# harshadms/galileo-sdr-sim

Measured on AMD Instinct MI355X. Metric: IQ Msamples/s (×real-time @2.6MS/s), 12-SV static E1B/C, 1/2/4/8 GPU, higher is better.
Workload: dtype f64 (NCO phases) + int16x2 (packed accumulate) -> int16 IQ; 1 GPU; M-SYN12: static-geometry 12-SV E1B/C, 1199 epochs x 260000 samples @2.6 MS/s per GPU (one independent scenario per rank); channels=12, chunk_samples=1024, walk_passes=1, synth_runs_max=1, chain_mismatch=0, pipeline_depth=2, window_mode=1, kernel_family=1, output_checksum=26e91314

## Files before the change

galileo-sdr-sim_amd/csrc/synth_api.cpp:

```cpp
#include <hip/hip_runtime.h>

#include <algorithm>
#include <cmath>
#include <cstdarg>
#include <cstddef>
#include <type_traits>
#include <cstdio>
#include <cstdlib>
#include <cstring>
#include <new>
#include <chrono>
#include <sched.h>
#include <time.h>
#include <vector>

#define GAL_SYNTH_NO_SIZED_MACROS 1
#include "nco_walk.h"
#include "synth_dev.h"
#include "e1_tables.inc"

static double rw_threshold_edge(double s)
{
    double g = 1.0;
    for (int u = 1; u <= 15; ++u) {
        const double us = (double)u * s;
        const double t = 1.0 - (us - std::floor(us));
        g = std::min(g, std::min(t, 1.0 - t));
    }
    return g;
}

static double rw_threshold_gap(double s)
{
    double T[15];
    for (int u = 1; u <= 15; ++u) {
        const double us = (double)u * s;
        const double t = 1.0 - (us - std::floor(us));
        int i = u - 1;
        while (i > 0 && T[i - 1] > t) { T[i] = T[i - 1]; --i; }
        T[i] = t;
    }
    double g = 1.0;
    for (int i = 1; i < 15; ++i) g = std::min(g, T[i] - T[i - 1]);
    return g;
}
static int rw_mode_of(double cs2)
{
    return (cs2 >= 0.74 && cs2 < 0.9999) ? 1 : (cs2 >= 0.0083 && cs2 <= 0.133) ? 2 : (cs2 > 0.133 && cs2 <= 0.266) ? 3
           : (cs2 > 0.266 && cs2 < 0.74) ? 4 : 0;
}
static constexpr double kRwMinGap = 1.0 / 128.0 + 4e-6;
static constexpr double kRwMinGapCboc = 1.0 / 64.0 + 4e-6;
#ifdef GAL_TEST_HOOKS
extern "C" double gal_hooks_rw_threshold_gap(double s) { return rw_threshold_gap(s); }
extern "C" double gal_hooks_rw_min_gap(void) { return kRwMinGap; }
#endif

extern "C" {
void galk_warm(hipStream_t st, int signal, double ratio);
void galk_warm_g(hipStream_t st);
int galk_launch_synth_g(const DevPlan *P, const DevPlan *Pd, int nch, int accumulate, const uint8_t *act, const int *nact,
                        uint32_t *iq, int e0, int ne, hipStream_t st);
void galk_launch_repair_g(const DevPlan *P, uint32_t *iq, int e0, hipStream_t st);
void galk_touch(hipStream_t st);
void galk_launch_walk_code(const DevPlan *P, hipStream_t st);
void galk_launch_walk_carr(const DevPlan *P, int first, hipStream_t st);
void galk_launch_carr_scan(const DevPlan *P, uint32_t tag, hipStream_t st);
size_t galk_scanm_status_bytes(int S, int legs);
void galk_launch_verify_carr(const DevPlan *P, hipStream_t st);
void galk_launch_verify_code(const DevPlan *P, hipStream_t st);
void galk_launch_pages(const DevPlan *P, hipStream_t st);
void galk_launch_publish(const DevPlan *P, int *h_ctr, void *h_state, uint32_t *h_flag, uint32_t seq, hipStream_t st);
int galk_scanm_blocks(int legs);
size_t galk_scanm_bytes(int S, int legs);
int galk_launch_synth(const DevPlan *P, const DevPlan *Pd, int nch, int accumulate, const uint8_t *act,
                      const int *nact, uint32_t *iq, int e0, int ne, hipStream_t st);
hipError_t galk_launch_iq(int format, const int16_t *in, uint64_t n_val, int shift, void *out, unsigned long long *sat, hipStream_t st);
hipError_t galk_launch_iq_noise(int format, const int16_t *in, uint64_t n_val, uint64_t first_sample, uint64_t seed, uint32_t stream,
                                uint32_t gain_q16, uint32_t sigma_q4, int shift, void *out, unsigned long long *sat, hipStream_t st);
}

namespace {

thread_local char g_err[512] = "";

int fail(int code, const char *fmt, ...)
{
    va_list ap;
    va_start(ap, fmt);
    vsnprintf(g_err, sizeof(g_err), fmt, ap);
    va_end(ap);
    return code;
}

#define HIP_TRY(expr)                                                                              \
    do {                                                                                           \
        hipError_t err__ = (expr);                                                                 \
        if (err__ != hipSuccess)                                                                   \
            return fail(GAL_E_DEVICE, "%s failed: %s (%s:%d)", #expr, hipGetErrorString(err__),   \
                        __FILE__, __LINE__);                                                       \
    } while (0)

int16_t g_cos[512], g_sin[512];
bool g_tables_ready = false;

void init_tables()
{
    if (g_tables_ready) return;
    for (int k = 0; k < 512; ++k) {
        int q;
        if (k < 128) q = kCosQ[k];
        else if (k < 256) q = -kCosQ[255 - k];
        else if (k < 384) q = -kCosQ[k - 256];
        else q = kCosQ[511 - k];
        g_cos[k] = (int16_t)q;
    }
    for (int k = 0; k < 512; ++k) g_sin[k] = g_cos[(k - 128) & 511];
    g_tables_ready = true;
}

constexpr int kKernelMaxChan = 12;
constexpr size_t kRunHostStagedBytes = 32u << 20;
constexpr int kActRow = 32;
// ... 25 lines not shown
        const double d = galnco::eff_step(dstep);
        const double mine = reset ? (restart ? p0 : start_in) : ph;
        const double full = (double)N * d;
        double y = mine + (full - std::trunc(full));
        y = y - std::trunc(y);
        const bool mixed = mine != 0.0 && d != 0.0 && ((mine < 0.0) != (d < 0.0));
        const bool crossed = !mixed || std::fabs(full) > std::fabs(mine);
        if (y != 0.0 && d != 0.0) {
            const bool neg = crossed ? d < 0.0 : mine < 0.0;
            if ((y < 0.0) != neg) y += neg ? -1.0 : 1.0;
        }
        ph = y;
        const bool use_root = reset || kind != 1;
        *pguess = mine;
        *gss_w = use_root ? (long long)e * N : ev_w;
        *gss_r = use_root ? mine : ev_r;
        int om;
        double rr;
        if (galnco::ideal_last_wrap(mine, d, N, &om, &rr)) {
            kind = 1;
            ev_w = (long long)e * N + om;
            ev_r = rr;
        } else if (reset) {
            kind = 1;
            ev_w = (long long)e * N;
            ev_r = mine;
        }
    }
};

struct StagedPlan {
    DevPlan P{};
    int n_groups = 0, all_first = 0, all_count = 0, n_exact_records = 0, nact_max = 0;
    std::vector<int> group_nch, group_kind;
    std::vector<int64_t> act_prefix;
    size_t o_plan = 0, o_act = 0, o_nact = 0, up_bytes = 0, total = 0;
    size_t o_cpx = 0, o_ancw = 0, zero_end = 0, o_clmw = 0, clmw_bytes = 0, o_scanm = 0, scanm_clear = 0;
    int R = 0, nchunks = 0;
    float ms_plan = 0.0f;
};

struct gal_synth {
    StagedPlan staged;
    bool staged_pending = false;
    gal_synth_cfg_t cfg{};
    int device = 0;
    int n_cu = 256;
    hipStream_t own_stream = nullptr;
    hipStream_t stream = nullptr;
    hipStream_t aux_stream = nullptr;
    hipStream_t walk_stream = nullptr;
    hipEvent_t ev_walk = nullptr;
    hipEvent_t ev_ver = nullptr;
    hipEvent_t ev_verc = nullptr;
    hipEvent_t ev_ctr = nullptr;
    hipEvent_t ev[4] = {nullptr, nullptr, nullptr, nullptr};
    hipEvent_t ev_prep = nullptr, ev_aux = nullptr;
    hipEvent_t ev_upd = nullptr;

    int *d_lut = nullptr;
    uint32_t *d_str = nullptr;
    DevPlan *d_plan = nullptr;
    char *h_up = nullptr;
    size_t h_up_bytes = 0;

    void *arena = nullptr;
    size_t arena_bytes = 0;
    DevPlan P{};
    DevPlan Pw{};
    bool planned = false;
    bool executed = false;
    bool in_flight = false;
    int n_groups = 0;
    std::vector<int> group_nch;
    std::vector<int> group_kind;
    int all_first = 0, all_count = 0;
    int n_exact_records = 0;
    uint8_t *d_act = nullptr;
    int *d_nact = nullptr;
    int nact_max = 0;
    uint32_t *last_iq = nullptr;
    int range_e0 = 0, range_ne = 0;
    void *own_iq = nullptr;
    size_t own_iq_bytes = 0;
    void *own_pin = nullptr;
    size_t own_pin_bytes = 0;
    int *h_ctr = nullptr;
    uint32_t *h_flag = nullptr;
    uint32_t seq = 0;
    uint32_t scan_tag = 0;
    size_t scanm_off = ~(size_t)0, scanm_clear = 0;
    int64_t legs_walked = 0, legs_translated = 0, n_fallbacks = 0;
    std::vector<int64_t> act_prefix;
    int64_t first_pass_legs = 0;
    gal_chan_state_t *h_state = nullptr;
    bool state_fetched = false;
    gal_synth_stats_t stats{};
    int enq_passes = kDefaultPasses;
    int small_need = 2;
    std::vector<double> rw_s0, rw_g0, rw_e0;
    std::vector<double> rw_rad;
    bool host_only = false;
    hipEvent_t ev_up0 = nullptr, ev_up1 = nullptr;
    bool upload_pending = false;
    bool upload_timed = false;
    bool upload_unordered = false;
    float ms_plan = 0.0f;
    double prev_wait_us = 0.0;
// ... 72 lines not shown

    int ndev = 0;
    if (hipGetDeviceCount(&ndev) != hipSuccess || ndev < 1)
        return fail(GAL_E_DEVICE, "no HIP device: the synthesis engine has no CPU fallback");
    create_stage("hipGetDeviceCount (HIP start-up)");
    int dev = cfg->device;
    if (dev < 0) HIP_TRY(hipGetDevice(&dev));
    if (dev >= ndev) return fail(GAL_E_INVAL, "device %d out of range (%d devices)", dev, ndev);
    HIP_TRY(hipSetDevice(dev));
    hipDeviceProp_t prop;
    HIP_TRY(hipGetDeviceProperties(&prop, dev));
    if (!strstr(prop.gcnArchName, "gfx950"))
        return fail(GAL_E_DEVICE, "device %d is %s; this library carries gfx950 code only", dev,
                    prop.gcnArchName);

    create_stage("set device + properties");
    gal_synth *h = new (std::nothrow) gal_synth();
    if (!h) return fail(GAL_E_NOMEM, "out of host memory");
    h->cfg = *cfg;
    h->device = dev;
    h->n_cu = prop.multiProcessorCount > 0 ? prop.multiProcessorCount : 256;
    auto bail = [&](int code) {
        gal_synth_destroy(h);
        return code;
    };
    {
        bool have = false;
        if (!(cfg->flags & GAL_CFG_SINGLE_STREAM)) {
            int least = 0, greatest = 0;
            hipStream_t ws = nullptr, as = nullptr;
            if (hipDeviceGetStreamPriorityRange(&least, &greatest) == hipSuccess &&
                hipStreamCreateWithPriority(&ws, hipStreamNonBlocking, greatest) == hipSuccess &&
                hipStreamCreateWithPriority(&as, hipStreamNonBlocking, greatest) == hipSuccess &&
                hipEventCreateWithFlags(&h->ev_walk, hipEventDisableTiming) == hipSuccess) {
                h->walk_stream = ws;
                h->aux_stream = as;
                have = true;
            } else {
                (void)hipGetLastError();
                if (ws) hipStreamDestroy(ws);
                if (as) hipStreamDestroy(as);
            }
        }
        if (!have && hipStreamCreateWithFlags(&h->aux_stream, hipStreamNonBlocking) != hipSuccess)
            return bail(fail(GAL_E_DEVICE, "hipStreamCreate failed"));
    }
    create_stage("streams");
    for (auto &e : h->ev)
        if (hipEventCreate(&e) != hipSuccess) return bail(fail(GAL_E_DEVICE, "hipEventCreate failed"));
    if (hipEventCreate(&h->ev_up0) != hipSuccess || hipEventCreate(&h->ev_up1) != hipSuccess ||
        hipEventCreateWithFlags(&h->ev_prep, hipEventDisableTiming) != hipSuccess ||
        hipEventCreateWithFlags(&h->ev_upd, hipEventDisableTiming) != hipSuccess ||
        hipEventCreateWithFlags(&h->ev_ver, hipEventDisableTiming) != hipSuccess ||
        hipEventCreateWithFlags(&h->ev_verc, hipEventDisableTiming) != hipSuccess ||
        hipEventCreateWithFlags(&h->ev_ctr, hipEventDisableTiming) != hipSuccess ||
        hipEventCreateWithFlags(&h->ev_aux, hipEventDisableTiming) != hipSuccess)
        return bail(fail(GAL_E_DEVICE, "hipEventCreate failed"));
    if (hipHostMalloc((void **)&h->h_ctr, (2 * CTR_COUNT + 16) * sizeof(int), hipHostMallocCoherent) != hipSuccess ||
        hipHostMalloc((void **)&h->h_state, sizeof(gal_chan_state_t) * GAL_ENGINE_MAX_CHAN,
                      hipHostMallocCoherent) != hipSuccess)
        return bail(fail(GAL_E_NOMEM, "pinned host allocation failed"));
    h->h_flag = (uint32_t *)(h->h_ctr + 2 * CTR_COUNT);
    *h->h_flag = 0;

    create_stage("events + pinned record");
    if (hipMalloc((void **)&h->d_lut, 2 * 512 * sizeof(int)) != hipSuccess ||
        hipMalloc((void **)&h->d_str, 50 * 512 * sizeof(uint32_t)) != hipSuccess)
        return bail(fail(GAL_E_NOMEM, "table allocation failed"));
    {
        std::vector<uint32_t> str(50 * 512, 0u);
        for (int prn = 0; prn < 50; ++prn)
            for (int hc = 0; hc < 2 * GAL_CODE_LEN; ++hc) {
                const int chip = hc >> 1;
                const uint32_t b = (kE1B[prn][chip >> 5] >> (chip & 31)) & 1u, c = (kE1C[prn][chip >> 5] >> (chip & 31)) & 1u;
                const uint32_t two = (b ^ c) | ((c ^ (uint32_t)(hc & 1)) << 1);
                str[prn * 512 + (hc >> 4)] |= two << (2 * (hc & 15));
            }
        if (hipMemcpy(h->d_str, str.data(), str.size() * sizeof(uint32_t), hipMemcpyHostToDevice) != hipSuccess)
            return bail(fail(GAL_E_DEVICE, "table upload failed"));
    }
    int lut[2 * 512];
    auto pair = [](int c, int s) {
        return (int)(((uint32_t)(uint16_t)(int16_t)(2 * s) << 16) | (uint32_t)(uint16_t)(int16_t)(2 * c));
    };
    if (cfg->flags & GAL_CFG_CBOC) {
        const double alpha = std::sqrt(10.0 / 11.0), beta = std::sqrt(1.0 / 11.0);
        for (int k = 0; k < 512; ++k) {
            lut[k] = pair((int)std::lround(alpha * (double)g_cos[k]), (int)std::lround(alpha * (double)g_sin[k]));
            lut[512 + k] = pair((int)std::lround(beta * (double)g_cos[k]), (int)std::lround(beta * (double)g_sin[k]));
        }
    } else {
        for (int k = 0; k < 512; ++k) lut[k] = lut[512 + k] = pair(g_cos[k], g_sin[k]);
    }
    if (hipMemcpy(h->d_lut, lut, sizeof(lut), hipMemcpyHostToDevice) != hipSuccess)
        return bail(fail(GAL_E_DEVICE, "table upload failed"));
    create_stage("tables (hipMalloc + uploads)");
    galk_warm(nullptr, (cfg->flags & GAL_CFG_CBOC) ? 1 : 0, 2.0 * 1.023e6 / cfg->sample_rate);
    {
        const double ratio = 2.0 * 1.023e6 / cfg->sample_rate;
        bool g_possible = false;
        for (const double f : {1.0 - 1e-4, 1.0, 1.0 + 1e-4}) {
            const int m = rw_mode_of(ratio * f);
            g_possible = g_possible || m != 0;
        }
        if (g_possible && !(cfg->flags & GAL_CFG_EXACT_REPLAY) && cfg->chunk_samples <= 0) galk_warm_g(nullptr);
    }
    create_stage("warm launches enqueued");
    if (h->walk_stream) {
        galk_touch(h->walk_stream);
        galk_touch(h->aux_stream);
        if (hipStreamSynchronize(h->walk_stream) != hipSuccess || hipStreamSynchronize(h->aux_stream) != hipSuccess) {
            gal_synth_destroy(h);
            return fail(GAL_E_DEVICE, "kernel launch failed on device %d: %s", dev, hipGetErrorString(hipGetLastError()));
        }
    }
    if (hipStreamSynchronize(nullptr) != hipSuccess) {
        gal_synth_destroy(h);
        return fail(GAL_E_DEVICE, "kernel launch failed on device %d: %s", dev, hipGetErrorString(hipGetLastError()));
    }
    create_stage("code objects loaded, streams used");
#ifdef GAL_TEST_HOOKS
    if (const char *env = getenv("GAL_SCAN_TAG0")) h->scan_tag = (uint32_t)strtoul(env, nullptr, 0);
#endif
    *out = h;
    return GAL_OK;
}

int gal_synth_destroy(gal_synth_t *h)
{
    if (!h) return GAL_OK;
    hipSetDevice(h->device);
    if (h->stream) hipStreamSynchronize(h->stream);
    if (h->arena) hipFree(h->arena);
    if (h->own_iq) hipFree(h->own_iq);
    if (h->own_pin) hipHostFree(h->own_pin);
    if (h->d_iq_sat) hipFree(h->d_iq_sat);
    if (h->d_lut) hipFree(h->d_lut);
    if (h->d_str) hipFree(h->d_str);
    if (h->h_up) hipHostFree(h->h_up);
    if (h->h_ctr) hipHostFree(h->h_ctr);
    if (h->h_state) hipHostFree(h->h_state);
    for (auto &e : h->ev)
        if (e) hipEventDestroy(e);
    if (h->ev_prep) hipEventDestroy(h->ev_prep);
    if (h->ev_upd) hipEventDestroy(h->ev_upd);
    if (h->ev_up0) hipEventDestroy(h->ev_up0);
    if (h->ev_up1) hipEventDestroy(h->ev_up1);
    if (h->ev_aux) hipEventDestroy(h->ev_aux);
    if (h->ev_walk) hipEventDestroy(h->ev_walk);
    if (h->ev_ver) hipEventDestroy(h->ev_ver);
    if (h->ev_verc) hipEventDestroy(h->ev_verc);
    if (h->ev_ctr) hipEventDestroy(h->ev_ctr);
    if (h->walk_stream) hipStreamDestroy(h->walk_stream);
    if (h->aux_stream) hipStreamDestroy(h->aux_stream);
    if (h->own_stream) hipStreamDestroy(h->own_stream);
    delete h;
    return GAL_OK;
}

int gal_synth_set_stream(gal_synth_t *h, void *hip_stream)
{
    if (!h) return fail(GAL_E_INVAL, "null handle");
    h->stream = hip_stream ? (hipStream_t)hip_stream : h->own_stream;
    return GAL_OK;
}

size_t gal_synth_output_bytes(const gal_synth_t *h)
{
    if (!h) return 0;
    if (h->staged_pending) return (size_t)h->staged.P.E * (size_t)h->staged.P.N * 4u;
    if (!h->planned) return 0;
    return (size_t)h->P.E * (size_t)h->P.N * 4u;
}

static size_t align_up(size_t v, size_t a) { return (v + a - 1) / a * a; }

static int commit_staged(gal_synth *h, const bool wait)
{
    StagedPlan &sp = h->staged;
    if (!h->host_only && sp.total > h->arena_bytes) {
        if (h->arena) hipFree(h->arena);
        h->arena = nullptr;
        h->arena_bytes = 0;
        if (hipMalloc(&h->arena, sp.total) != hipSuccess) return fail(GAL_E_NOMEM, "hipMalloc of %zu bytes failed", sp.total);
        h->arena_bytes = sp.total;
        h->scanm_off = ~(size_t)0;
    }
    char *const base = (char *)h->arena;
    DevPlan &P = sp.P;
    {
        auto rb = [&](auto *&ptr) { ptr = (std::remove_reference_t<decltype(ptr)>)(base + (size_t)(uintptr_t)ptr); };
        rb(P.page_init); rb(P.init_ix); rb(P.state_in); rb(P.state_out); rb(P.prn); rb(P.flags); rb(P.ib0); rb(P.x0); rb(P.p0);
        rb(P.cstep); rb(P.dstep); rb(P.page_next); rb(P.page_cur); rb(P.flip_in); rb(P.pguess); rb(P.gss_w); rb(P.gss_r);
        rb(P.anc_w); rb(P.anc_r); rb(P.clm_w); rb(P.clm_r); rb(P.pend); rb(P.verified); rb(P.dirty); rb(P.risk); rb(P.marg);
        rb(P.shift); rb(P.tpos); rb(P.tdir); rb(P.scanm); rb(P.cp_x); rb(P.cp_p); rb(P.cp_ib); rb(P.ctr); rb(P.gflist);
    }
    h->P = P;
    h->d_plan = (DevPlan *)(base + sp.o_plan);
    h->d_act = (uint8_t *)(base + sp.o_act);
    h->d_nact = (int *)(base + sp.o_nact);
    h->n_groups = sp.n_groups; h->all_first = sp.all_first; h->all_count = sp.all_count; h->n_exact_records = sp.n_exact_records;
    h->group_nch = std::move(sp.group_nch);
    h->group_kind = std::move(sp.group_kind);
    h->act_prefix = std::move(sp.act_prefix);
    h->nact_max = sp.nact_max;
// ... 471 lines not shown
int gal_synth_plan_async(gal_synth_t *h, const gal_chan_epoch_t *params, int32_t n_epochs, const gal_chan_state_t *state_in)
{
    return plan_impl(h, params, n_epochs, state_in, false);
}

#ifdef GAL_TEST_HOOKS
static gal_synth *g_host_plan = nullptr;
double gal_hooks_plan_host_ms(const gal_synth_cfg_t *cfg, const gal_chan_epoch_t *params, int32_t n_epochs, const gal_chan_state_t *state_in,
                              int32_t reps)
{
    gal_synth *&g = g_host_plan;
    if (g) {
        free(g->h_up);
        delete g;
        g = nullptr;
    }
    if (!cfg || !params) return -1.0;
    g = new gal_synth();
    g->cfg = *cfg;
    g->host_only = true;
    init_tables();
    double best = 1e30;
    for (int r = 0; r < (reps > 0 ? reps : 1); ++r) {
        const auto t0 = std::chrono::steady_clock::now();
        if (plan_impl(g, params, n_epochs, state_in, false) != GAL_OK) return -1.0;
        best = std::min(best, std::chrono::duration<double, std::milli>(std::chrono::steady_clock::now() - t0).count());
    }
    return best;
}
const void *gal_hooks_plan_host_array(const char *name)
{
    const gal_synth *g = g_host_plan;
    if (!g || !g->planned || !name) return nullptr;
    const DevPlan &P = g->P;
    const struct { const char *n; const void *p; } tab[] = {
        {"prn", P.prn}, {"flags", P.flags}, {"ib0", P.ib0}, {"x0", P.x0}, {"p0", P.p0}, {"cstep", P.cstep}, {"dstep", P.dstep},
        {"page_next", P.page_next}, {"pguess", P.pguess}, {"gss_w", P.gss_w}, {"gss_r", P.gss_r}, {"init_ix", P.init_ix},
        {"page_init", P.page_init}, {"state_in", P.state_in}, {"act", g->d_act}, {"nact", g->d_nact}};
    for (const auto &t : tab)
        if (!strcmp(t.n, name)) return g->h_up + (size_t)(uintptr_t)t.p;
    if (!strcmp(name, "family")) return (const void *)(uintptr_t)(1 + P.fam);
    if (!strcmp(name, "groups")) return (const void *)(uintptr_t)(1 + g->n_groups);
    if (!strcmp(name, "search")) return (const void *)(uintptr_t)(1 + P.rw_search);
    if (!strcmp(name, "form")) return (const void *)(uintptr_t)(1 + P.rw);
    return nullptr;
}
#endif

static int enqueue_synth(gal_synth *h, uint32_t *iq, bool verify_here)
{
    if (verify_here && h->P.fam == 1 && h->nact_max != 0) {
        DevPlan Pv = h->Pw;
        if (h->stats.synth_runs > 1) Pv.ver_mod = 1, Pv.ver_rem = 0;
        galk_launch_verify_carr(&Pv, h->stream);
        galk_launch_verify_code(&Pv, h->stream);
    }
    if (h->nact_max == 0) {
        HIP_TRY(hipMemsetAsync(iq, 0, (size_t)h->range_ne * (size_t)h->P.N * 4u, h->stream));
        return GAL_OK;
    }
    const bool overflow_set = h->P.fam == 0 && h->all_count > 0;
    const int g_first = overflow_set ? h->all_first : 0, g_count = overflow_set ? h->all_count : h->n_groups;
    DevPlan Px = h->P;
    if (h->P.fam == 1 || overflow_set) Px.rw = 0;
    for (int k = 0; k < g_count; ++k) {
        const int g = g_first + k;
        const uint8_t *act = h->d_act + (size_t)g * h->P.E * kActRow;
        const int *nact = h->d_nact + (size_t)g * h->P.E;
        const bool on_g = h->P.fam == 1 && h->group_kind[g] == 1;
        const int rc = on_g ? galk_launch_synth_g(&h->P, h->d_plan, h->group_nch[g], k > 0, act, nact, iq, h->range_e0, h->range_ne, h->stream)
                            : galk_launch_synth(h->P.fam == 1 || overflow_set ? &Px : &h->P, h->d_plan, h->group_nch[g], k > 0, act, nact, iq,
                                                h->range_e0, h->range_ne, h->stream);
        if (rc) return fail(GAL_E_INVAL, "no synthesis kernel for %d channels per group", h->group_nch[g]);
    }
    if (h->P.fam == 1) {
        HIP_TRY(hipEventRecord(h->ev[3], h->stream));
        galk_launch_repair_g(&h->P, iq, h->range_e0, h->stream);
    }
    HIP_TRY(hipGetLastError());
    return GAL_OK;
}

static int ensure_committed(gal_synth *h)
{
    if (!h->staged_pending) return GAL_OK;
    if (h->in_flight) return fail(GAL_E_STATE, "gal_synth_execute while a batch is in flight: call gal_synth_finish first");
    HIP_TRY(hipSetDevice(h->device));
    return commit_staged(h, false);
}

int gal_synth_execute(gal_synth_t *h, int16_t *iq_dev)
{
    if (!h) return fail(GAL_E_INVAL, "gal_synth_execute: null argument");
    if (const int rc = ensure_committed(h)) return rc;
    if (!h->planned) return fail(GAL_E_STATE, "gal_synth_execute before gal_synth_plan");
    return gal_synth_execute_range(h, iq_dev, 0, h->P.E);
}

int gal_synth_execute_range(gal_synth_t *h, int16_t *iq_dev, int32_t first_epoch, int32_t n_epochs)
{
    if (!h || !iq_dev) return fail(GAL_E_INVAL, "gal_synth_execute: null argument");
    if (const int rc = ensure_committed(h)) return rc;
    if (!h->planned) return fail(GAL_E_STATE, "gal_synth_execute before gal_synth_plan");
    if (first_epoch < 0 || n_epochs < 1 || first_epoch + n_epochs > h->P.E)
        return fail(GAL_E_INVAL, "gal_synth_execute_range: epochs [%d, %d) outside the planned batch of %d", first_epoch,
                    first_epoch + n_epochs, h->P.E);
    if (h->in_flight)
        return fail(GAL_E_STATE, "gal_synth_execute while a batch is in flight: call gal_synth_finish first");
    if (((uintptr_t)iq_dev) & 15) return fail(GAL_E_INVAL, "iq_dev must be 16-byte aligned");
    HIP_TRY(hipSetDevice(h->device));
    if (h->executed && (first_epoch != h->range_e0 || n_epochs != h->range_ne)) h->enq_passes = std::max(h->enq_passes, kDefaultPasses);
    h->range_e0 = first_epoch;
    h->range_ne = n_epochs;
    h->Pw = h->P;
    h->Pw.E = first_epoch + n_epochs;
    h->Pw.LEGS = h->Pw.E * h->P.W;
    h->Pw.tr_e0 = first_epoch;
    h->Pw.tr_e1 = first_epoch + n_epochs;
    h->Pw.cp_e0 = first_epoch;
    h->Pw.ver_mod = (h->cfg.flags & GAL_CFG_VERIFY_SAMPLED) ? kVerifyRotation : 1;
#ifdef GAL_TEST_HOOKS
    if (const char *env = getenv("GAL_VERIFY_MOD")) h->Pw.ver_mod = atoi(env) > 0 ? atoi(env) : h->Pw.ver_mod;
#endif
    h->Pw.ver_rem = (int)((h->seq + 1u) % (uint32_t)h->Pw.ver_mod);
    hipStream_t st = handle_stream(h);
    if (!st) return fail(GAL_E_DEVICE, "hipStreamCreate failed");
    const DevPlan *P = &h->Pw;
    hipStream_t ws = h->walk_stream ? h->walk_stream : st;
    if (h->upload_unordered) {
        if (ws != st) HIP_TRY(hipStreamWaitEvent(ws, h->ev_upd, 0));
        h->upload_unordered = false;
    }
    HIP_TRY(hipEventRecord(h->ev[0], ws));
    HIP_TRY(hipEventRecord(h->ev_prep, ws));
    const bool code_first = h->Pw.E * 8 < 256 && h->aux_stream && h->aux_stream != ws;
    if (code_first) {
        HIP_TRY(hipStreamWaitEvent(h->aux_stream, h->ev_prep, 0));
        galk_launch_walk_code(P, h->aux_stream);
        galk_launch_pages(P, h->aux_stream);
        HIP_TRY(hipEventRecord(h->ev_aux, h->aux_stream));
    }
    int n_passes = h->enq_passes;
#ifdef GAL_TEST_HOOKS
    if (const char *env = getenv("GAL_WALK_PASSES")) n_passes = atoi(env) > 0 ? atoi(env) : n_passes;
#endif
    h->first_pass_legs = h->act_prefix[h->Pw.E] * h->P.W;
    if (h->scan_tag > 0xFFF00000u) {
        HIP_TRY(hipMemsetAsync((char *)h->P.scanm, 0, h->scanm_clear, ws));
        h->scan_tag = 0;
    }
    for (int pass = 0; pass < n_passes; ++pass) {
        galk_launch_walk_carr(P, pass == 0, ws);
        if (pass == 0 && ws != st) HIP_TRY(hipEventRecord(h->ev_ctr, ws));
        galk_launch_carr_scan(P, ++h->scan_tag, ws);
    }
    if (!code_first) {
        HIP_TRY(hipStreamWaitEvent(h->aux_stream, h->ev_prep, 0));
        galk_launch_walk_code(P, h->aux_stream);
        galk_launch_pages(P, h->aux_stream);
        HIP_TRY(hipEventRecord(h->ev_aux, h->aux_stream));
    }
    bool verify_beside = h->P.fam == 1 && ws != st && h->nact_max != 0;
#ifdef GAL_TEST_HOOKS
    const bool no_verify = getenv("GAL_G_NOVERIFY") != nullptr;
    if (no_verify) verify_beside = false;
#else
    const bool no_verify = false;
#endif
    if (ws != st) {
        HIP_TRY(hipEventRecord(h->ev_walk, ws));
        HIP_TRY(hipStreamWaitEvent(st, h->ev_walk, 0));
        if (verify_beside) {
            galk_launch_verify_carr(P, ws);
            HIP_TRY(hipEventRecord(h->ev_ver, ws));
            HIP_TRY(hipStreamWaitEvent(h->aux_stream, h->ev_ctr, 0));
            galk_launch_verify_code(P, h->aux_stream);
            HIP_TRY(hipEventRecord(h->ev_verc, h->aux_stream));
        }
    }
    HIP_TRY(hipStreamWaitEvent(st, h->ev_aux, 0));
    HIP_TRY(hipEventRecord(h->ev[1], st));
    int rc = enqueue_synth(h, (uint32_t *)iq_dev, !verify_beside && !no_verify);
    if (rc) return rc;
    HIP_TRY(hipEventRecord(h->ev[2], st));
    if (verify_beside) {
        HIP_TRY(hipStreamWaitEvent(st, h->ev_ver, 0));
        HIP_TRY(hipStreamWaitEvent(st, h->ev_verc, 0));
    }
    h->seq += 1;
    if (h->seq == 0) h->seq = 1;
    galk_launch_publish(P, h->h_ctr, h->h_state, h->h_flag, h->seq, st);
    h->state_fetched = true;
    h->last_iq = (uint32_t *)iq_dev;
    h->stats.synth_runs = 1;
    h->executed = true;
    h->in_flight = true;
    return GAL_OK;
}

size_t gal_synth_stats_size(void) { return sizeof(gal_synth_stats_t); }

static void copy_stats(const gal_synth *h, void *stats, size_t stats_bytes)
{
    if (stats) memcpy(stats, &h->stats, std::min(stats_bytes, sizeof(gal_synth_stats_t)));
}

static constexpr size_t kStatsBytesV02 = 40;
static_assert(offsetof(gal_synth_stats_t, kernel_family) == kStatsBytesV02, "gal_synth_stats_t 0.2 ends in front of kernel_family");

int gal_synth_finish(gal_synth_t *h, gal_chan_state_t *state_out, gal_synth_stats_t *stats)
{
    return gal_synth_finish_n(h, state_out, stats, kStatsBytesV02);
}

int gal_synth_finish_n(gal_synth_t *h, gal_chan_state_t *state_out, void *stats, size_t stats_bytes)
{
    if (!h) return fail(GAL_E_INVAL, "null handle");
    if (!h->executed) return fail(GAL_E_STATE, "gal_synth_finish before gal_synth_execute");
    h->in_flight = false;
    HIP_TRY(hipSetDevice(h->device));
    hipStream_t st = handle_stream(h);
    if (!st) return fail(GAL_E_DEVICE, "hipStreamCreate failed");
    const DevPlan *P = &h->Pw;
    {
        const uint32_t want = h->seq;
        const auto t_begin = std::chrono::steady_clock::now();
        unsigned spins = 0;
        double waited_us = 0.0;
        const double nap_until_us = 0.7 * h->prev_wait_us - 150.0;
        while (__atomic_load_n(h->h_flag, __ATOMIC_ACQUIRE) != want) {
            const bool look = (++spins & 255u) == 0;
            if (!look) {
                __builtin_ia32_pause();
                continue;
            }
            waited_us = std::chrono::duration<double, std::micro>(std::chrono::steady_clock::now() - t_begin).count();
            bool napped = false;
            if (waited_us >= 50.0) {
                if (waited_us < nap_until_us) {
                    timespec ts{0, 50000};
                    nanosleep(&ts, nullptr);
// ... 325 lines not shown
```

galileo-sdr-sim_amd/csrc/synth_kernels.hip:

```cpp
#include <hip/hip_runtime.h>
#include <stdint.h>

#include "nco_walk.h"
#include "synth_dev.h"
#include "synth_common.h"

using namespace galnco;
using namespace galdev;

#if !defined(GAL_TU)
#define GAL_TU_WALK 1
#define GAL_TU_SYNTH 1
#define GAL_TU_FAMILY(k) 1
#else
#define GAL_TU_WALK (GAL_TU == 0)
#define GAL_TU_SYNTH (GAL_TU != 0)
#define GAL_TU_FAMILY(k) (GAL_TU == (k))
#endif

#ifndef GAL_WALK_PRIO
#define GAL_WALK_PRIO 3
#endif
#if GAL_WALK_PRIO > 0
#define GAL_WALK_SETPRIO() __builtin_amdgcn_s_setprio(GAL_WALK_PRIO)
#else
#define GAL_WALK_SETPRIO() ((void)0)
#endif

#ifdef GAL_TEST_HOOKS
#define GAL_HOOK_BAD_LEG 5
#endif

#if GAL_TU_WALK
__device__ __forceinline__ double shfl_up1_f64(double v)
{
    const uint64_t u = d2u(v);
    const uint32_t lo = (uint32_t)__shfl_up((int)(uint32_t)u, 1), hi = (uint32_t)__shfl_up((int)(uint32_t)(u >> 32), 1);
    return u2d(((uint64_t)hi << 32) | lo);
}

__global__ void k_walk_code(DevPlan P)
{
    GAL_WALK_SETPRIO();
    const int Wc = P.Wc;
    const int t = blockIdx.x * blockDim.x + threadIdx.x;
    if (t >= P.E * P.S * Wc) return;
    const int k = t & (Wc - 1);
    const int se = t / Wc;
    const int s = se / P.E;
    const int idx = (se - s * P.E) * P.S + s;
    if (P.prn[idx] <= 0) return;
    double *cpx = P.cp_x + (size_t)idx * P.CP1;
    uint32_t *cpi = P.cp_ib + (size_t)idx * P.CP1;
    const double c = P.cstep[idx];
// ... 197 lines not shown
                for (int q = 0; q < 8; ++q) v[q] = P.dstep[(size_t)(e2 + q) * P.S + s];
                bool still = true;
#pragma unroll
                for (int q = 0; q < 8; ++q) still = still && v[q] == 0.0;
                if (!still) break;
                e2 += 8;
            }
            const long long skip_to = e2 * P.N;
            cur = skip_to < A ? skip_to : A;
            continue;
        }
        const WalkOut o = carr_walk_track(p, d, 1.0 / __builtin_fabs(d), n, n, n, [](int, double) {});
        if (o.last_w >= 0) {
            lw = cur + o.last_w;
            lr = o.last_r;
        }
        mg = o.margin < mg ? o.margin : mg;
        if (!tdir && o.tdir) {
            tdir = o.tdir;
            tpos = cur + o.tpos;
        }
        p = o.p;
        cur = seg_end;
    }
    int n = P.N - w * L;
    n = n > L ? L : n;
    const double d = P.dstep[idx];
    double *cpp = P.cp_p + (size_t)idx * P.CP1 + (size_t)w * P.Lc;
    const WalkOut o = e < P.cp_e0 ? carr_walk_track(p, d, 1.0 / __builtin_fabs(d), n, n, n, [](int, double) {})
                                  : carr_walk_track(p, d, 1.0 / __builtin_fabs(d), n, P.R, 0, [&](int c, double v) { cpp[c] = v; });
    if (o.last_w >= 0) {
        lw = A + o.last_w;
        lr = o.last_r;
    }
    if (w == P.W - 1) P.cp_p[(size_t)idx * P.CP1 + P.nchunks] = o.p;
    P.pend[li] = o.p;
    P.clm_w[li] = lw;
    P.clm_r[li] = lr;
    P.marg[li] = o.margin < mg ? o.margin : mg;
    if (!tdir && o.tdir) {
        tdir = o.tdir;
        tpos = A + o.tpos;
    }
    P.tdir[li] = (int8_t)tdir;
    P.tpos[li] = tpos;
    P.dirty[li] = 0;
    P.risk[li] = 0;
    if (!first) {
        const uint64_t m = __builtin_amdgcn_ballot_w64(true);
        if ((int)(threadIdx.x & 63) == __builtin_ctzll(m)) atomicAdd(&P.ctr[CTR_WALKS], __builtin_popcountll(m));
    }
}

__device__ __forceinline__ void verify_carr_leg(const DevPlan &P, const int s, const int i)
{
    const int e = i / P.W, w = i - e * P.W;
    if (e < P.cp_e0) return;
    const int idx = e * P.S + s;
    if (P.prn[idx] <= 0) return;
    const int L = P.Lc * P.R;
    int n = P.N - w * L;
    n = n > L ? L : n;
    if (n <= 0) return;
    const double d = P.dstep[idx];
    const double *cpp = P.cp_p + (size_t)idx * P.CP1 + (size_t)w * P.Lc;
    int bad = 0;
    const WalkOut o = carr_walk_track(cpp[0], d, 1.0 / __builtin_fabs(d), n, P.R, 0, [&](int c, double v) { bad += cpp[c] != v; });
    bad += cpp[(n + P.R - 1) / P.R] != o.p;
    if (bad) atomicAdd(&P.ctr[CTR_MISMATCH], bad);
}

__global__ void k_verify_carr(DevPlan P)
{
    if (P.ctr[CTR_UNVERIFIED] != 0) return;
    const int mod = P.ver_mod > 1 ? P.ver_mod : 1;
    const int per_slot = (P.LEGS + mod - 1) / mod;
    const int nsel = per_slot * P.S;
    int t = blockIdx.x * blockDim.x + threadIdx.x;
    if (t < nsel) {
        const int s = t / per_slot;
        const int i = (t - s * per_slot) * mod + P.ver_rem;
        if (i < P.LEGS) verify_carr_leg(P, s, i);
        return;
    }
    t -= nsel;
    const int total = P.LEGS * P.S;
    if (mod == 1 || t * 8 >= total) return;
#pragma unroll 1
    for (int q = 0; q < 8 && t * 8 + q < total; ++q) {
        const int li = t * 8 + q;
        if (!P.risk[li] || li % P.LEGS % mod == P.ver_rem) continue;
        const int s = li / P.LEGS;
        verify_carr_leg(P, s, li - s * P.LEGS);
    }
}

__global__ void k_verify_code(DevPlan P)
{
    const int Wc = P.Wc;
    const int t = blockIdx.x * blockDim.x + threadIdx.x;
    if (t >= P.E * P.S * Wc) return;
    const int k = t & (Wc - 1);
    const int se = t / Wc;
    const int s = se / P.E;
    const int e = se - s * P.E;
    if (e < P.cp_e0) return;
    const int idx = e * P.S + s;
    if (P.prn[idx] <= 0) return;
    const int mod = P.ver_mod > 1 ? P.ver_mod : 1;
    if (mod > 1 && (e * Wc + k) % mod != P.ver_rem) return;
    const int Lk = P.Lkc;
    const int n0 = k * Lk * P.R;
    if (n0 >= P.N) return;
    int n1 = (k + 1) * Lk * P.R;
    n1 = n1 > P.N ? P.N : n1;
    const double *cpx = P.cp_x + (size_t)idx * P.CP1 + (size_t)k * Lk;
    const uint32_t *cpi = P.cp_ib + (size_t)idx * P.CP1 + (size_t)k * Lk;
    const double c = P.cstep[idx];
    const uint32_t w0 = cpi[0];
    const int fl0 = (int)(w0 >> 16);
    int bad = 0;
    if (k == 0) bad += d2u(cpx[0]) != d2u(P.x0[idx]) || w0 != (uint32_t)P.ib0[idx];
    const CodeEnd end = code_walk(cpx[0], (int)(w0 & 0xffffu), c, 1.0 / c, n1 - n0, P.R, [&](int ci, double x, int ib, int fl) {
        bad += d2u(cpx[ci]) != d2u(x) || cpi[ci] != ((uint32_t)ib | ((uint32_t)(fl | fl0) << 16));
    });
    const int nck = (n1 - n0 + P.R - 1) / P.R;
    bad += d2u(cpx[nck]) != d2u(end.x) || cpi[nck] != ((uint32_t)end.ibit | ((uint32_t)(end.flipped | fl0) << 16));
    if (n1 >= P.N) bad += P.flip_in[idx] != (uint8_t)(end.flipped | fl0);
    if (bad) atomicAdd(&P.ctr[CTR_MISMATCH], bad);
}

struct ClaimState {
    int kind;
    long long w;
    double r;
};

struct LegRec {
    bool act, root, dirty, hw;
    int tdir;
    long long A, aw, cw;
    double ar, cr, known;
};

__device__ __forceinline__ LegRec leg_load(const DevPlan &P, int s, int i, double start0)
{
    LegRec L;
    const int e = i / P.W, w = i - e * P.W;
    const int idx = e * P.S + s;
    const size_t li = (size_t)s * P.LEGS + i;
    L.act = P.prn[idx] > 0;
    const uint32_t fl = P.flags[idx];
    L.root = L.act && w == 0 && (e == 0 || (fl & GAL_CH_RESTART));
    L.known = (fl & GAL_CH_RESTART) ? P.p0[idx] : start0;
    L.A = (long long)e * P.N + (long long)w * (P.Lc * P.R);
    L.aw = P.anc_w[li];
    L.ar = P.anc_r[li];
    L.cw = P.clm_w[li];
    L.cr = P.clm_r[li];
    L.hw = L.act && L.cw >= 0;
    L.tdir = P.tdir[li];
    L.dirty = L.act && P.dirty[li] != 0;
    return L;
}

#define GAL_U52 2.220446049250313e-16

__device__ __forceinline__ int d_residue(double D) { return (int)((long long)(D * 4503599627370496.0) & 3LL); }

__device__ __forceinline__ double tie_flip(double t, int tdir)
{
    return (tdir != 0 && (d_residue(t) & 1)) ? t - (double)tdir * GAL_U52 : t;
}

struct DMap {
    int isconst;
    double K;
    double c[4];
};

__device__ __forceinline__ double dmap_pick(const DMap &f, int r)
{
// ... 1388 lines not shown

    {
        const double *const q_cpx = Pd->cp_x, *const q_cpp = Pd->cp_p;
        const uint32_t *const q_cpi = Pd->cp_ib;
        double ex[NCH], ep[NCH];
        uint32_t ei[NCH];
#pragma unroll
        for (int j = 0; j < NCH; ++j) {
            const size_t cp = (size_t)ixs[j] * G.CP1 + c + 1;
            ex[j] = q_cpx[cp];
            ep[j] = q_cpp[cp];
            ei[j] = q_cpi[cp];
        }
        int bad = 0;
#define GAL_CHECK(j)                                                                  \
    if (j < NCH && j < nact) {                                                        \
        const uint32_t v = ei[j < NCH ? j : 0];                                       \
        bad += d2u(ch##j.y) != d2u(2.0 * ex[j < NCH ? j : 0]);                        \
        { double pm = ep[j < NCH ? j : 0]; GAL_MIRROR_BITS(pm, ds##j)                 \
          bad += ch##j.p != pm; }  \
        bad += (ch##j.st & 0x3ffu) != ((v & 0x1ffu) | ((v >> 16) << 9));              \
    }
        GAL_CH_LIST(GAL_CHECK)
#undef GAL_CHECK
#undef GAL_MIRROR_BITS
#undef GAL_HI
        if (c == 0 && e > 0) {
#define GAL_LINK(j)                                                                                  \
    if (j < NCH && j < nact) {                                                                       \
        const int idx = ix##j;                                                                       \
        if (!(Pd->flags[idx] & GAL_CH_RESTART)) {                                                    \
            const double p_in = q_cpp[(size_t)idx * G.CP1];                                          \
            const double p_prev = q_cpp[(size_t)(idx - G.S) * G.CP1 + G.nchunks];                    \
            bad += d2u(p_in) != d2u(p_prev);                                                         \
        }                                                                                            \
    }
            GAL_CH_LIST(GAL_LINK)
#undef GAL_LINK
        }
        if (bad) atomicAdd(&Pd->ctr[CTR_MISMATCH], bad);
    }
}

#endif

#if GAL_TU_WALK

extern "C" void galk_launch_walk_code(const DevPlan *P, hipStream_t st)
{
    const int n = P->E * P->S * P->Wc;
    hipLaunchKernelGGL(k_walk_code, dim3((n + 63) / 64), dim3(64), 0, st, *P);
}

extern "C" void galk_launch_verify_carr(const DevPlan *P, hipStream_t st)
{
    const int mod = P->ver_mod > 1 ? P->ver_mod : 1;
    const int nsel = (P->LEGS + mod - 1) / mod * P->S;
    const int n = nsel + (mod > 1 ? (P->LEGS * P->S + 7) / 8 : 0);
    hipLaunchKernelGGL(k_verify_carr, dim3((n + 255) / 256), dim3(256), 0, st, *P);
}

extern "C" void galk_launch_verify_code(const DevPlan *P, hipStream_t st)
{
    const int n = P->E * P->S * P->Wc;
    hipLaunchKernelGGL(k_verify_code, dim3((n + 63) / 64), dim3(64), 0, st, *P);
}

extern "C" void galk_launch_walk_carr(const DevPlan *P, int first, hipStream_t st)
{
    const int n = P->LEGS * P->S;
    hipLaunchKernelGGL(k_walk_carr, dim3((n + 63) / 64), dim3(64), 0, st, *P, first);
}

#ifdef GAL_TEST_HOOKS
extern "C" int galk_scanm_stamps(unsigned long long *out, int reset)
{
    if (out && hipMemcpyFromSymbol(out, HIP_SYMBOL(g_scanm_stamp), sizeof(g_scanm_stamp)) != hipSuccess) return -1;
    if (reset) {
        void *d = nullptr;
        if (hipGetSymbolAddress(&d, HIP_SYMBOL(g_scanm_stamp)) != hipSuccess || hipMemset(d, 0, sizeof(g_scanm_stamp)) != hipSuccess) return -1;
    }
    return 0;
}
#endif

static int scanm_lpb()
{
#ifdef GAL_TEST_HOOKS
    if (const char *e = getenv("GAL_SCAN_BLOCK_LEGS")) {
        const int v = atoi(e);
        if (v >= 1 && v <= SCANM_THREADS) return v;
    }
#endif
    return SCANM_THREADS;
}

extern "C" int galk_scanm_blocks(int legs) { return (legs + scanm_lpb() - 1) / scanm_lpb(); }

extern "C" size_t galk_scanm_status_bytes(int S, int legs) { return 256 + ((size_t)S * galk_scanm_blocks(legs) * 4 + 255) / 256 * 256 * 2; }
extern "C" size_t galk_scanm_bytes(int S, int legs)
{
    const size_t SB = (size_t)S * galk_scanm_blocks(legs);
    return galk_scanm_status_bytes(S, legs) + ((SB * 4 + 255) / 256 * 256) * 2 + ((SB * 8 + 255) / 256 * 256) * 3 + ((SB * 32 + 255) / 256 * 256) + 4096;
}

extern "C" void galk_launch_carr_scan(const DevPlan *P, uint32_t tag, hipStream_t st)
{
    ScanM M;
    M.lpb = scanm_lpb();
    M.B = galk_scanm_blocks(P->LEGS);
    M.Bs = galk_scanm_blocks(P->LEGS_all > P->LEGS ? P->LEGS_all : P->LEGS);
    M.tag = tag ? tag : 1u;
    M.nap = 1;
#ifdef GAL_TEST_HOOKS
    if (const char *e = getenv("GAL_SCANM_NAP")) M.nap = atoi(e);
#endif
    const size_t SB = (size_t)P->S * M.Bs;
    char *p = (char *)P->scanm;
// ... 131 lines not shown
```

Baseline: 295,200 Msamples/s.

## Fuse carrier and code verify into one kernel with split sub-runs

Merges the separate carrier-phase and code-phase verification kernels into a single launch on the walk stream, dropping the aux-stream verify, its extra events and cross-stream waits. Each leg or code window is also split into 2^q sub-runs verified by separate threads, with the count chosen from the total chunk count. This exposes more parallelism and shortens the per-thread serial walk, and it starts at cp_e0 so threads are not spent on skipped epochs. In exchange each sub-run re-seeds from the stored checkpoint, which adds a boundary check, and the code verify now waits on ev_aux instead of overlapping with it.

```diff
diff --git a/galileo-sdr-sim_amd/csrc/synth_api.cpp b/galileo-sdr-sim_amd/csrc/synth_api.cpp
--- a/galileo-sdr-sim_amd/csrc/synth_api.cpp
+++ b/galileo-sdr-sim_amd/csrc/synth_api.cpp
@@ -67,8 +67,7 @@
 void galk_launch_walk_carr(const DevPlan *P, int first, hipStream_t st);
 void galk_launch_carr_scan(const DevPlan *P, uint32_t tag, hipStream_t st);
 size_t galk_scanm_status_bytes(int S, int legs);
-void galk_launch_verify_carr(const DevPlan *P, hipStream_t st);
-void galk_launch_verify_code(const DevPlan *P, hipStream_t st);
+void galk_launch_verify(const DevPlan *P, hipStream_t st);
 void galk_launch_pages(const DevPlan *P, hipStream_t st);
 void galk_launch_publish(const DevPlan *P, int *h_ctr, void *h_state, uint32_t *h_flag, uint32_t seq, hipStream_t st);
 int galk_scanm_blocks(int legs);
@@ -200,8 +199,6 @@
     hipStream_t walk_stream = nullptr;
     hipEvent_t ev_walk = nullptr;
     hipEvent_t ev_ver = nullptr;
-    hipEvent_t ev_verc = nullptr;
-    hipEvent_t ev_ctr = nullptr;
     hipEvent_t ev[4] = {nullptr, nullptr, nullptr, nullptr};
     hipEvent_t ev_prep = nullptr, ev_aux = nullptr;
     hipEvent_t ev_upd = nullptr;
@@ -380,8 +377,6 @@
         hipEventCreateWithFlags(&h->ev_prep, hipEventDisableTiming) != hipSuccess ||
         hipEventCreateWithFlags(&h->ev_upd, hipEventDisableTiming) != hipSuccess ||
         hipEventCreateWithFlags(&h->ev_ver, hipEventDisableTiming) != hipSuccess ||
-        hipEventCreateWithFlags(&h->ev_verc, hipEventDisableTiming) != hipSuccess ||
-        hipEventCreateWithFlags(&h->ev_ctr, hipEventDisableTiming) != hipSuccess ||
         hipEventCreateWithFlags(&h->ev_aux, hipEventDisableTiming) != hipSuccess)
         return bail(fail(GAL_E_DEVICE, "hipEventCreate failed"));
     if (hipHostMalloc((void **)&h->h_ctr, (2 * CTR_COUNT + 16) * sizeof(int), hipHostMallocCoherent) != hipSuccess ||
@@ -477,8 +472,6 @@
     if (h->ev_aux) hipEventDestroy(h->ev_aux);
     if (h->ev_walk) hipEventDestroy(h->ev_walk);
     if (h->ev_ver) hipEventDestroy(h->ev_ver);
-    if (h->ev_verc) hipEventDestroy(h->ev_verc);
-    if (h->ev_ctr) hipEventDestroy(h->ev_ctr);
     if (h->walk_stream) hipStreamDestroy(h->walk_stream);
     if (h->aux_stream) hipStreamDestroy(h->aux_stream);
     if (h->own_stream) hipStreamDestroy(h->own_stream);
@@ -1056,8 +1049,7 @@
     if (verify_here && h->P.fam == 1 && h->nact_max != 0) {
         DevPlan Pv = h->Pw;
         if (h->stats.synth_runs > 1) Pv.ver_mod = 1, Pv.ver_rem = 0;
-        galk_launch_verify_carr(&Pv, h->stream);
-        galk_launch_verify_code(&Pv, h->stream);
+        galk_launch_verify(&Pv, h->stream);
     }
     if (h->nact_max == 0) {
         HIP_TRY(hipMemsetAsync(iq, 0, (size_t)h->range_ne * (size_t)h->P.N * 4u, h->stream));
@@ -1155,7 +1147,6 @@
     }
     for (int pass = 0; pass < n_passes; ++pass) {
         galk_launch_walk_carr(P, pass == 0, ws);
-        if (pass == 0 && ws != st) HIP_TRY(hipEventRecord(h->ev_ctr, ws));
         galk_launch_carr_scan(P, ++h->scan_tag, ws);
     }
     if (!code_first) {
@@ -1175,11 +1166,9 @@
         HIP_TRY(hipEventRecord(h->ev_walk, ws));
         HIP_TRY(hipStreamWaitEvent(st, h->ev_walk, 0));
         if (verify_beside) {
-            galk_launch_verify_carr(P, ws);
+            HIP_TRY(hipStreamWaitEvent(ws, h->ev_aux, 0));
+            galk_launch_verify(P, ws);
             HIP_TRY(hipEventRecord(h->ev_ver, ws));
-            HIP_TRY(hipStreamWaitEvent(h->aux_stream, h->ev_ctr, 0));
-            galk_launch_verify_code(P, h->aux_stream);
-            HIP_TRY(hipEventRecord(h->ev_verc, h->aux_stream));
         }
     }
     HIP_TRY(hipStreamWaitEvent(st, h->ev_aux, 0));
@@ -1187,10 +1176,7 @@
     int rc = enqueue_synth(h, (uint32_t *)iq_dev, !verify_beside && !no_verify);
     if (rc) return rc;
     HIP_TRY(hipEventRecord(h->ev[2], st));
-    if (verify_beside) {
-        HIP_TRY(hipStreamWaitEvent(st, h->ev_ver, 0));
-        HIP_TRY(hipStreamWaitEvent(st, h->ev_verc, 0));
-    }
+    if (verify_beside) HIP_TRY(hipStreamWaitEvent(st, h->ev_ver, 0));
     h->seq += 1;
     if (h->seq == 0) h->seq = 1;
     galk_launch_publish(P, h->h_ctr, h->h_state, h->h_flag, h->seq, st);
diff --git a/galileo-sdr-sim_amd/csrc/synth_kernels.hip b/galileo-sdr-sim_amd/csrc/synth_kernels.hip
--- a/galileo-sdr-sim_amd/csrc/synth_kernels.hip
+++ b/galileo-sdr-sim_amd/csrc/synth_kernels.hip
@@ -1,5 +1,7 @@
 #include <hip/hip_runtime.h>
 #include <stdint.h>
+#include <stdio.h>
+#include <stdlib.h>
 
 #include "nco_walk.h"
 #include "synth_dev.h"
@@ -303,82 +305,119 @@
     }
 }
 
-__device__ __forceinline__ void verify_carr_leg(const DevPlan &P, const int s, const int i)
+struct VerCut {
+    int qs, qcs;
+    int blocksA, blocksB;
+    int hook_chain, hook_e, hook_c;
+};
+
+#define VERIFY_THREADS 256
+
+__device__ __forceinline__ void verify_carr_run(const DevPlan &P, const VerCut &V, const int s, const int e, const int c0, const int c1)
+{
+    if (c1 <= c0) return;
+    const int idx = e * P.S + s;
+    if (P.prn[idx] <= 0) return;
+    const int n0 = c0 * P.R;
+    int n = c1 * P.R;
+    n = (n > P.N ? P.N : n) - n0;
+    const double d = P.dstep[idx];
+    const double *cpp = P.cp_p + (size_t)idx * P.CP1 + c0;
+#ifdef GAL_TEST_HOOKS
+    const int hc = (V.hook_chain == 1 && s == 0 && e == V.hook_e) ? V.hook_c - c0 : -1;
+    auto ld = [&](int c) { return c == hc ? u2d(d2u(cpp[c]) ^ (1ull << 32)) : cpp[c]; };
+#else
+    auto ld = [&](int c) { return cpp[c]; };
+#endif
+    int bad = 0;
+    if (c0 == 0 && e > 0 && !(P.flags[idx] & GAL_CH_RESTART)) bad += d2u(ld(0)) != d2u(cpp[-(ptrdiff_t)P.S * P.CP1 + P.nchunks]);
+    const WalkOut o = carr_walk_track(ld(0), d, 1.0 / __builtin_fabs(d), n, P.R, 0, [&](int c, double v) { bad += ld(c) != v; });
+    bad += ld(c1 - c0) != o.p;
+    if (bad) atomicAdd(&P.ctr[CTR_MISMATCH], bad);
+}
+
+__device__ __forceinline__ void verify_carr_leg_run(const DevPlan &P, const VerCut &V, const int s, const int i, const int j)
 {
     const int e = i / P.W, w = i - e * P.W;
     if (e < P.cp_e0) return;
+    int nck = P.nchunks - w * P.Lc;
+    nck = nck > P.Lc ? P.Lc : nck;
+    verify_carr_run(P, V, s, e, w * P.Lc + ((j * nck) >> V.qs), w * P.Lc + (((j + 1) * nck) >> V.qs));
+}
+
+__device__ __forceinline__ void verify_code_run(const DevPlan &P, const VerCut &V, const int s, const int e, const int c0, const int c1)
+{
+    if (c1 <= c0) return;
     const int idx = e * P.S + s;
     if (P.prn[idx] <= 0) return;
-    const int L = P.Lc * P.R;
-    int n = P.N - w * L;
-    n = n > L ? L : n;
-    if (n <= 0) return;
-    const double d = P.dstep[idx];
-    const double *cpp = P.cp_p + (size_t)idx * P.CP1 + (size_t)w * P.Lc;
-    int bad = 0;
-    const WalkOut o = carr_walk_track(cpp[0], d, 1.0 / __builtin_fabs(d), n, P.R, 0, [&](int c, double v) { bad += cpp[c] != v; });
-    bad += cpp[(n + P.R - 1) / P.R] != o.p;
-    if (bad) atomicAdd(&P.ctr[CTR_MISMATCH], bad);
-}
-
-__global__ void k_verify_carr(DevPlan P)
-{
-    if (P.ctr[CTR_UNVERIFIED] != 0) return;
-    const int mod = P.ver_mod > 1 ? P.ver_mod : 1;
-    const int per_slot = (P.LEGS + mod - 1) / mod;
-    const int nsel = per_slot * P.S;
-    int t = blockIdx.x * blockDim.x + threadIdx.x;
-    if (t < nsel) {
-        const int s = t / per_slot;
-        const int i = (t - s * per_slot) * mod + P.ver_rem;
-        if (i < P.LEGS) verify_carr_leg(P, s, i);
-        return;
-    }
-    t -= nsel;
-    const int total = P.LEGS * P.S;
-    if (mod == 1 || t * 8 >= total) return;
-#pragma unroll 1
-    for (int q = 0; q < 8 && t * 8 + q < total; ++q) {
-        const int li = t * 8 + q;
-        if (!P.risk[li] || li % P.LEGS % mod == P.ver_rem) continue;
-        const int s = li / P.LEGS;
-        verify_carr_leg(P, s, li - s * P.LEGS);
-    }
-}
-
-__global__ void k_verify_code(DevPlan P)
-{
-    const int Wc = P.Wc;
-    const int t = blockIdx.x * blockDim.x + threadIdx.x;
-    if (t >= P.E * P.S * Wc) return;
-    const int k = t & (Wc - 1);
-    const int se = t / Wc;
-    const int s = se / P.E;
-    const int e = se - s * P.E;
-    if (e < P.cp_e0) return;
-    const int idx = e * P.S + s;
-    if (P.prn[idx] <= 0) return;
-    const int mod = P.ver_mod > 1 ? P.ver_mod : 1;
-    if (mod > 1 && (e * Wc + k) % mod != P.ver_rem) return;
-    const int Lk = P.Lkc;
-    const int n0 = k * Lk * P.R;
-    if (n0 >= P.N) return;
-    int n1 = (k + 1) * Lk * P.R;
+    const int n0 = c0 * P.R;
+    int n1 = c1 * P.R;
     n1 = n1 > P.N ? P.N : n1;
-    const double *cpx = P.cp_x + (size_t)idx * P.CP1 + (size_t)k * Lk;
-    const uint32_t *cpi = P.cp_ib + (size_t)idx * P.CP1 + (size_t)k * Lk;
+    const double *cpx = P.cp_x + (size_t)idx * P.CP1 + c0;
+    const uint32_t *cpi = P.cp_ib + (size_t)idx * P.CP1 + c0;
+#ifdef GAL_TEST_HOOKS
+    const int hc = (V.hook_chain == 2 && s == 0 && e == V.hook_e) ? V.hook_c - c0 : -1;
+    auto ldx = [&](int c) { return c == hc ? d2u(cpx[c]) ^ (1ull << 32) : d2u(cpx[c]); };
+#else
+    auto ldx = [&](int c) { return d2u(cpx[c]); };
+#endif
     const double c = P.cstep[idx];
     const uint32_t w0 = cpi[0];
     const int fl0 = (int)(w0 >> 16);
+    const uint64_t xs = ldx(0);
     int bad = 0;
-    if (k == 0) bad += d2u(cpx[0]) != d2u(P.x0[idx]) || w0 != (uint32_t)P.ib0[idx];
-    const CodeEnd end = code_walk(cpx[0], (int)(w0 & 0xffffu), c, 1.0 / c, n1 - n0, P.R, [&](int ci, double x, int ib, int fl) {
-        bad += d2u(cpx[ci]) != d2u(x) || cpi[ci] != ((uint32_t)ib | ((uint32_t)(fl | fl0) << 16));
+    if (c0 == 0) bad += xs != d2u(P.x0[idx]) || w0 != (uint32_t)P.ib0[idx];
+    const CodeEnd end = code_walk(u2d(xs), (int)(w0 & 0xffffu), c, 1.0 / c, n1 - n0, P.R, [&](int ci, double x, int ib, int fl) {
+        bad += ldx(ci) != d2u(x) || cpi[ci] != ((uint32_t)ib | ((uint32_t)(fl | fl0) << 16));
     });
-    const int nck = (n1 - n0 + P.R - 1) / P.R;
-    bad += d2u(cpx[nck]) != d2u(end.x) || cpi[nck] != ((uint32_t)end.ibit | ((uint32_t)(end.flipped | fl0) << 16));
+    const int nck = c1 - c0;
+    bad += ldx(nck) != d2u(end.x) || cpi[nck] != ((uint32_t)end.ibit | ((uint32_t)(end.flipped | fl0) << 16));
     if (n1 >= P.N) bad += P.flip_in[idx] != (uint8_t)(end.flipped | fl0);
     if (bad) atomicAdd(&P.ctr[CTR_MISMATCH], bad);
+}
+
+__global__ __launch_bounds__(VERIFY_THREADS) void k_verify(DevPlan P, VerCut V)
+{
+    if (P.ctr[CTR_UNVERIFIED] != 0) return;
+    const int s = blockIdx.y;
+    const int mod = P.ver_mod > 1 ? P.ver_mod : 1;
+    const int leg0 = P.cp_e0 * P.W;
+    int bx = blockIdx.x;
+    if (bx < V.blocksA) {
+        const int u = bx * VERIFY_THREADS + threadIdx.x;
+        int first = leg0 - leg0 % mod + P.ver_rem;
+        first += first < leg0 ? mod : 0;
+        const int i = first + (u >> V.qs) * mod;
+        if (i < P.LEGS) verify_carr_leg_run(P, V, s, i, u & ((1 << V.qs) - 1));
+        return;
+    }
+    bx -= V.blocksA;
+    if (bx < V.blocksB) {
+        const int t = bx * VERIFY_THREADS + threadIdx.x;
+        const uint8_t *risk = P.risk + (size_t)s * P.LEGS;
+#pragma unroll 1
+        for (int q = 0; q < 8 && t * 8 + q < P.LEGS; ++q) {
+            const int i = t * 8 + q;
+            if (i < leg0 || !risk[i] || i % mod == P.ver_rem) continue;
+#pragma unroll 1
+            for (int j = 0; j < (1 << V.qs); ++j) verify_carr_leg_run(P, V, s, i, j);
+        }
+        return;
+    }
+    bx -= V.blocksB;
+    {
+        const int u = bx * VERIFY_THREADS + threadIdx.x;
+        const int j = u & ((1 << V.qcs) - 1);
+        const int ek = u >> V.qcs;
+        const int k = ek & (P.Wc - 1);
+        const int e = P.cp_e0 + ek / P.Wc;
+        if (e >= P.E) return;
+        if (mod > 1 && (e * P.Wc + k) % mod != P.ver_rem) return;
+        int nck = P.nchunks - k * P.Lkc;
+        nck = nck > P.Lkc ? P.Lkc : nck;
+        if (nck <= 0) return;
+        verify_code_run(P, V, s, e, k * P.Lkc + ((j * nck) >> V.qcs), k * P.Lkc + (((j + 1) * nck) >> V.qcs));
+    }
 }
 
 struct ClaimState {
@@ -1873,18 +1912,48 @@
     hipLaunchKernelGGL(k_walk_code, dim3((n + 63) / 64), dim3(64), 0, st, *P);
 }
 
-extern "C" void galk_launch_verify_carr(const DevPlan *P, hipStream_t st)
+static int verify_log2_runs(long long chunks, int leg_chunks, int run_max, int run_min)
+{
+    const long long lanes = 1024ll * 64 * 4;
+    long long m = (chunks + lanes - 1) / lanes;
+    m = m > run_max ? run_max : m < run_min ? run_min : m;
+    int q = 0;
+    while (q < 6 && ((leg_chunks + (1 << q) - 1) >> q) > m) ++q;
+    return q;
+}
+
+extern "C" void galk_launch_verify(const DevPlan *P, hipStream_t st)
 {
     const int mod = P->ver_mod > 1 ? P->ver_mod : 1;
-    const int nsel = (P->LEGS + mod - 1) / mod * P->S;
-    const int n = nsel + (mod > 1 ? (P->LEGS * P->S + 7) / 8 : 0);
-    hipLaunchKernelGGL(k_verify_carr, dim3((n + 255) / 256), dim3(256), 0, st, *P);
-}
-
-extern "C" void galk_launch_verify_code(const DevPlan *P, hipStream_t st)
-{
-    const int n = P->E * P->S * P->Wc;
-    hipLaunchKernelGGL(k_verify_code, dim3((n + 63) / 64), dim3(64), 0, st, *P);
+    const int ne = P->E - P->cp_e0;
+    if (ne <= 0) return;
+    int run_c = 8, run_k = 16;
+    VerCut V{};
+#ifdef GAL_TEST_HOOKS
+    if (const char *e = getenv("GAL_VERIFY_RUN")) {
+        int a = 0, b = 0;
+        const int got = sscanf(e, "%d,%d", &a, &b);
+        if (got >= 1 && a > 0) run_c = a;
+        if (got >= 2 && b > 0) run_k = b;
+    }
+    if (const char *e = getenv("GAL_VERIFY_CORRUPT")) {
+        int a = 0, b = 0, c = 0;
+        if (sscanf(e, "%d,%d,%d", &a, &b, &c) == 3) V.hook_chain = a, V.hook_e = b, V.hook_c = c;
+    }
+    const bool forced = getenv("GAL_VERIFY_RUN") != nullptr;
+#else
+    const bool forced = false;
+#endif
+    const long long chunks = (long long)ne * P->S * P->nchunks / mod;
+    V.qs = verify_log2_runs(chunks, P->Lc, run_c, forced ? run_c : 2);
+    V.qcs = verify_log2_runs(chunks, P->Lkc, run_k, forced ? run_k : 4);
+    const int legs_sel = (ne * P->W + mod - 1) / mod;
+    const long long nA = (long long)legs_sel << V.qs;
+    const long long nC = ((long long)ne * P->Wc) << V.qcs;
+    V.blocksA = (int)((nA + VERIFY_THREADS - 1) / VERIFY_THREADS);
+    V.blocksB = mod > 1 ? ((P->LEGS + 7) / 8 + VERIFY_THREADS - 1) / VERIFY_THREADS : 0;
+    const int blocksC = (int)((nC + VERIFY_THREADS - 1) / VERIFY_THREADS);
+    hipLaunchKernelGGL(k_verify, dim3(V.blocksA + V.blocksB + blocksC, P->S), dim3(VERIFY_THREADS), 0, st, *P, V);
 }
 
 extern "C" void galk_launch_walk_carr(const DevPlan *P, int first, hipStream_t st)
```

Measured after the change: 296,100 Msamples/s (median of 4 runs). Within noise of the previous version (+0.3%).
